# WeChatCV/WeDetect

Hardware: AMD Instinct MI355X
Metric: images/s at 640x640 (WeDetect-Base image tower + 80-class similarity + top-k/NMS) (higher is better)
Workload: dtype f32-equivalent: fp32 operands carried as fp16 hi+lo pairs, 3 fp16-MFMA passes per product, fp32 accumulate (fp16x3); similarity GEMM, dwconv, LN, post-process native f32

## Files before the change

__graft_entry__.py:

```python
import os
import sys

ROOT = os.path.dirname(os.path.abspath(__file__))
if ROOT not in sys.path:
    sys.path.insert(0, ROOT)


def build() -> None:
    from wedetect_amd import build as wb
    wb.build()
    import wedetect_amd.lib as lib
    import wedetect_amd.feed
    import wedetect_amd.tile
    import wedetect_amd.views
    import wedetect_amd.fold
    import wedetect_amd.best
    import wedetect_amd.sparse
    import wedetect_amd.topn
    import wedetect_amd.groups
    import wedetect_amd.exemplar
    import wedetect_amd.tune
    import wedetect_amd.track
    import wedetect_amd.detector
    import oracle.postprocess
    import oracle.ref_cpu
    print("built and loaded", lib.LIB_PATH)


def smoke() -> None:
    import numpy as np
    import torch
    from oracle import postprocess as opp
    from oracle import ref_cpu as orc
    from wedetect_amd import weights as W
    from wedetect_amd.arch import get_arch
    from wedetect_amd.engine import ImageTower
    from wedetect_amd.pack import pack

    assert torch.cuda.is_available(), "smoke() needs a HIP device"
    torch.cuda.set_device(0)
    arch, b, hw, npr = "tiny", 2, 128, 64
    sd_np = W.make_state_dict(arch, num_prompts=npr)
    tower = ImageTower(arch, pack(sd_np, arch), b, hw, hw)
    imgs = W.make_images(b, hw, hw)
    embed, boxes = tower.features(torch.from_numpy(imgs).cuda())
# ... 27 lines not shown
```

wedetect_amd/build.py:

```python
from __future__ import annotations

import os
import subprocess
import sys

HERE = os.path.dirname(os.path.abspath(__file__))
ROOT = os.path.dirname(HERE)
CSRC = os.path.join(HERE, "csrc")
LIB = os.path.join(HERE, "libwedetect_hip.so")
SOURCES = ["abi.hip", "conv_gemm.hip", "similarity_grouped.hip", "split_gemm.hip", "split_gemm_pre.hip", "split_gemm_p8.hip", "split_gemm_p4.hip", "split_gemm_conv.hip", "split_gemm_conv3.hip", "split_gemm_mlp.hip", "split_gemm_mlpw.hip", "probe.hip", "stem.hip", "elementwise.hip", "preprocess.hip", "text.hip", "bricks.hip", "evaluate.hip", "det_eval.hip", "postprocess.hip", "feed.hip", "tile.hip", "views.hip", "fold.hip", "best.hip", "sparse.hip", "topn.hip", "groups.hip", "exemplar.hip", "tune.hip", "track.hip"]
PUBLIC_HEADERS = ["wedetect_hip.h", "wedetect_hip_feed.h", "wedetect_hip_tile.h", "wedetect_hip_views.h", "wedetect_hip_fold.h", "wedetect_hip_best.h", "wedetect_hip_sparse.h", "wedetect_hip_topn.h", "wedetect_hip_groups.h", "wedetect_hip_exemplar.h", "wedetect_hip_tune.h", "wedetect_hip_track.h"]
HIPCC = os.environ.get("HIPCC", "/opt/rocm/bin/hipcc")
FLAGS = ["--offload-arch=gfx950", "-O3", "-std=c++17", "-fPIC", "-Wall", "-Wno-unused-function", "-Wno-inline-asm",
         "-I", os.path.join(ROOT, "include"), "-I", CSRC]
for _d in os.environ.get("WD_EXTRA_DEFINES", "").split():
    FLAGS.append("-D" + _d)
if os.environ.get("WD_DEBUG_ABLATIONS") == "1":
    FLAGS.append("-DWD_DEBUG_ABLATIONS")


def _headers():
    return [os.path.join(CSRC, f) for f in os.listdir(CSRC) if f.endswith(".h")] + [os.path.join(ROOT, "include", h) for h in PUBLIC_HEADERS]


def source_hash() -> str:
    import hashlib
    h = hashlib.sha256()
    files = sorted(os.path.join(CSRC, f) for f in os.listdir(CSRC) if f.endswith((".hip", ".h")))
    for f in files + [os.path.join(ROOT, "include", h) for h in PUBLIC_HEADERS]:
        h.update(os.path.basename(f).encode())
        h.update(open(f, "rb").read())
    return h.hexdigest()


# ... 112 lines not shown
```

wedetect_amd/csrc/split_gemm_mlpw.hip:

```cpp
#include <stdlib.h>
#include "split_epi_oct.h"
#include "split_mlp_epi.h"

namespace {

template <int C>
struct MW {
  static constexpr int H = 4 * C, BM = 128, HC = 128, NCH = H / HC;
  static constexpr int KT = 64, NKT = C / KT;
  static constexpr int XSLOT = BM * 256, NSLOT = 3;
  static constexpr int HOFF = NSLOT * XSLOT;
  static constexpr int LDS = HOFF + BM * 512;
  static constexpr int TN2 = C / 128;
  static constexpr int S1 = C / 16, S2 = H / 16;
  static_assert(C % 128 == 0 && NKT >= 2 && LDS <= 160 * 1024, "shape");
  static_assert(4 * 32 * EPI_LDT * 4 <= HOFF, "the epilogue patches reuse the ring");
};

struct MwArgs {
  const unsigned char* a;
  const unsigned char* w1;
  const unsigned char* w2;
  const float* b1;
  const float* b2;
// ... 40 lines not shown
    asm volatile("global_load_dwordx4 %0, %2, %3\n\tglobal_load_dwordx4 %1, %2, %3 offset:1024"
                 : "=&v"(hi), "=&v"(lo) : "v"(lane16), "s"(base) : "memory");
}
template <bool SAFE>
__device__ __forceinline__ void mw_bload(f32x4& d, unsigned voff, const float* base) {
  if constexpr (SAFE)
    asm volatile("s_nop 4\n\tglobal_load_dwordx4 %0, %1, %2" : "=&v"(d) : "v"(voff), "s"(base) : "memory");
  else
    asm volatile("global_load_dwordx4 %0, %1, %2" : "=&v"(d) : "v"(voff), "s"(base) : "memory");
}
#define MW_WAIT8_(N, A0, A1, A2, A3, A4, A5, A6, A7) \
  asm volatile("s_waitcnt vmcnt(" #N ")" : "+v"(A0), "+v"(A1), "+v"(A2), "+v"(A3), "+v"(A4), "+v"(A5), "+v"(A6), "+v"(A7) :: "memory")
#ifdef MW_EXPERIMENT_ALL0
#define MW_WAIT8(N, ...) MW_WAIT8_(0, __VA_ARGS__)
#else
#define MW_WAIT8(N, ...) MW_WAIT8_(N, __VA_ARGS__)
#endif

template <int C, int ABL = 0, bool PERSIST = false, bool FOLD = false>
__global__ void __launch_bounds__(256) fused_mlp_wide_kernel(const MwArgs q) {
  using P = MW<C>;
  constexpr int TN2 = P::TN2, NKT = P::NKT;
  static_assert(NKT % 2 == 0 && NKT >= 4, "K tiles alternate between two W1 fragment buffers");
  extern __shared__ __attribute__((aligned(16))) unsigned char smem_raw[];
  const int t = threadIdx.x, lane = t & 63;
  const int wave = __builtin_amdgcn_readfirstlane(t >> 6);
  int first_blk, seg_o, last_blk, seg_e;
  if (PERSIST) {
    const int b = blockIdx.x, xcd = b & 7, slot = b >> 3, per = gridDim.x >> 3;
    const long long t0 = (long long)q.nblk * xcd / 8, t1 = (long long)q.nblk * (xcd + 1) / 8;
    const long long units = (t1 - t0) * P::NCH;
    const long long u0 = t0 * P::NCH + units * slot / per, u1 = t0 * P::NCH + units * (slot + 1) / per;
    first_blk = (int)(u0 / P::NCH); seg_o = (int)(u0 - (long long)first_blk * P::NCH);
    last_blk = (int)(u1 / P::NCH); seg_e = (int)(u1 - (long long)last_blk * P::NCH);
  } else {
    int tile = blockIdx.x;
    const int nwg = gridDim.x, xcd = tile & 7, idx = tile >> 3;
    const int qq = nwg >> 3, r = nwg & 7;
    tile = (xcd < r ? xcd * (qq + 1) : r * (qq + 1) + (xcd - r) * qq) + idx;
    first_blk = tile; seg_o = 0; last_blk = tile + 1; seg_e = 0;
  }
  const int has_head = seg_e > 0, has_tail = seg_o > 0;
  const int full0 = first_blk + has_tail, nfull = last_blk - full0;
  const int nseg = has_head + nfull + has_tail;
  unsigned lds0 = (unsigned)(size_t)(__attribute__((address_space(3))) unsigned char*)smem_raw;

// ... 13 lines not shown
  const int r = lane & 31, hsel = lane >> 5, f = r & 15;
  const int xb = r * 256 + (((2 * hsel) ^ f) << 4);
  const int hb = r * 512 + (((2 * hsel) ^ f) << 4);
  const unsigned char* hbuf = smem_raw + P::HOFF;

  const unsigned lane16 = (unsigned)lane * 16u;
  const unsigned char* w1w_ = q.w1 + (size_t)wave * (P::S1 * 2048);
  const unsigned char* w2w_ = q.w2 + (size_t)(TN2 * wave) * (P::S2 * 2048);
  const unsigned char *w1w = w1w_, *w2w = w2w_;
  const unsigned bvoff = (unsigned)hsel * 16u;
  const float* b1p = q.b1 + wave * 32;
  const float* u1p = FOLD ? q.ln_u + wave * 32 : nullptr;

  using I0 = std::integral_constant<int, 0>;
  using I1 = std::integral_constant<int, 1>;

  for (int sg = 0; sg < nseg; ++sg) {
  const bool is_head = has_head && sg == 0;
  const bool is_tail = has_tail && sg == nseg - 1;
  const int blk = is_head ? last_blk : (is_tail ? first_blk : full0 + sg - has_head);
  const int c0 = is_tail ? seg_o : 0, c1 = is_head ? seg_e : P::NCH;
  const int m0 = blk * P::BM;
  arow = q.a + (size_t)m0 * (C * 4);
  MW_BARRIER();

  f32x16 out[4][TN2];
  if (PERSIST && is_tail) {
    const int prev = blockIdx.x - 8;
    if (t == 0) {
      while (__hip_atomic_load(q.flag + prev, __ATOMIC_RELAXED, __HIP_MEMORY_SCOPE_AGENT) != 1u) __builtin_amdgcn_s_sleep(8);
      __builtin_amdgcn_fence(__ATOMIC_ACQUIRE, "agent");
    }
    __syncthreads();
    const unsigned char* sb = reinterpret_cast<const unsigned char*>(q.park) + (size_t)prev * (4 * TN2 * 4 * 4096);
    const unsigned toff = (unsigned)t * 16u;
#pragma unroll
    for (int i = 0; i < 4; ++i) {
      f32x4 v[TN2][4];
#pragma unroll
      for (int jn = 0; jn < TN2; ++jn)
#pragma unroll
        for (int g = 0; g < 4; ++g) {
          MW_OPAQUE(sb);
          v[jn][g] = *reinterpret_cast<const f32x4*>(sb + toff);
          sb += 4096;
        }
// ... 23 lines not shown
  h8 wh[2][4], wl[2][4];
  h8 vh[2][TN2], vl[2][TN2];
  f32x4 bq[4];
  f32x4 uq[4] = {};
  typedef float f32x2_ __attribute__((ext_vector_type(2)));
  f32x2_ st[4] = {};

  auto load_w1_tile = [&](int j, int kt, int buf) {
    if ((ABL & 8) && (j > c0 || kt > 1)) return;
    const unsigned char* b = w1w + (size_t)(4 * j) * (P::S1 * 2048) + kt * 8192;
#pragma unroll
    for (int s = 0; s < 4; ++s) mw_wload<PERSIST>(wh[buf][s], wl[buf][s], lane16, b + s * 2048);
  };
  auto load_w2_step = [&](int S, int buf) {
    if ((ABL & 8) && S > 1) return;
    const unsigned char* b = w2w + (size_t)S * 2048;
#pragma unroll
    for (int jn = 0; jn < TN2; ++jn) mw_wload<PERSIST>(vh[buf][jn], vl[buf][jn], lane16, b + (size_t)jn * (P::S2 * 2048));
  };
  auto load_bias = [&](int j) {
    const float* b = b1p + j * P::HC;
#pragma unroll
    for (int g = 0; g < 4; ++g) mw_bload<PERSIST>(bq[g], bvoff, b + 8 * g);
    if constexpr (FOLD) {
      const float* u = u1p + j * P::HC;
#pragma unroll
      for (int g = 0; g < 4; ++g) mw_bload<PERSIST>(uq[g], bvoff, u + 8 * g);
    }
  };

  MW_OPAQUE(arow); MW_OPAQUE(w1w); MW_OPAQUE(w2w); MW_OPAQUE(b1p); MW_OPAQUE(lds0);
  issue_x(0, 0);
  issue_x(1, 1);
  load_w1_tile(c0, 0, 0);
  load_w1_tile(c0, 1, 1);
  load_bias(c0);
  if constexpr (FOLD) {
    const float* sp = q.ln_stats + 2 * (size_t)m0;
    MW_OPAQUE(sp);
#pragma unroll
    for (int i = 0; i < 4; ++i) {
      const unsigned so = (unsigned)(32 * i + r) * 8u;
      if constexpr (PERSIST) asm volatile("s_nop 4\n\tglobal_load_dwordx2 %0, %1, %2" : "=&v"(st[i]) : "v"(so), "s"(sp) : "memory");
      else asm volatile("global_load_dwordx2 %0, %1, %2" : "=&v"(st[i]) : "v"(so), "s"(sp) : "memory");
    }
    asm volatile("s_waitcnt vmcnt(0)" : "+v"(st[0]), "+v"(st[1]), "+v"(st[2]), "+v"(st[3]) :: "memory");
  } else {
    asm volatile("s_waitcnt vmcnt(0)" ::: "memory");
  }

  for (int j = c0; j < c1; ++j) {
    const int jn1 = j + 1 < c1 ? j + 1 : j;
    MW_OPAQUE(arow); MW_OPAQUE(w1w); MW_OPAQUE(w2w); MW_OPAQUE(b1p); MW_OPAQUE(lds0);
    f32x16 g1[4];
#pragma unroll
    for (int i = 0; i < 4; ++i)
#pragma unroll
      for (int e = 0; e < 16; ++e) g1[i][e] = 0.0f;

    auto ktile = [&](auto kt_c, auto buf_c, int slot) {
      constexpr int KT_ = decltype(kt_c)::value, BUF = decltype(buf_c)::value;
      if (!(ABL & 2)) {
#ifdef MW_EXPERIMENT_TILE_WAIT
        MW_WAIT8(MW_EXPERIMENT_TILE_WAIT, wh[BUF][0], wl[BUF][0], wh[BUF][1], wl[BUF][1], wh[BUF][2], wl[BUF][2], wh[BUF][3], wl[BUF][3]);
#else
        if constexpr (KT_ == 0 && TN2 == 2 && FOLD) MW_WAIT8(20, wh[BUF][0], wl[BUF][0], wh[BUF][1], wl[BUF][1], wh[BUF][2], wl[BUF][2], wh[BUF][3], wl[BUF][3]);
        else if constexpr (KT_ == 0 && TN2 == 2) MW_WAIT8(16, wh[BUF][0], wl[BUF][0], wh[BUF][1], wl[BUF][1], wh[BUF][2], wl[BUF][2], wh[BUF][3], wl[BUF][3]);
        else if constexpr (KT_ <= 1 && FOLD) MW_WAIT8(24, wh[BUF][0], wl[BUF][0], wh[BUF][1], wl[BUF][1], wh[BUF][2], wl[BUF][2], wh[BUF][3], wl[BUF][3]);
        else if constexpr (KT_ <= 1) MW_WAIT8(20, wh[BUF][0], wl[BUF][0], wh[BUF][1], wl[BUF][1], wh[BUF][2], wl[BUF][2], wh[BUF][3], wl[BUF][3]);
        else if constexpr (KT_ == NKT - 1) MW_WAIT8(8, wh[BUF][0], wl[BUF][0], wh[BUF][1], wl[BUF][1], wh[BUF][2], wl[BUF][2], wh[BUF][3], wl[BUF][3]);
        else MW_WAIT8(16, wh[BUF][0], wl[BUF][0], wh[BUF][1], wl[BUF][1], wh[BUF][2], wl[BUF][2], wh[BUF][3], wl[BUF][3]);
#endif
      }
      if (!(ABL & 4)) MW_BARRIER();
      {
        int s2 = slot + 2;
        if (s2 >= P::NSLOT) s2 -= P::NSLOT;
        issue_x(KT_ + 2 < NKT ? KT_ + 2 : KT_ + 2 - NKT, s2);
      }
      const unsigned char* xs = smem_raw + slot * P::XSLOT;
      const unsigned char* wnext = w1w + (size_t)(4 * j) * (P::S1 * 2048) + (KT_ + 2) * 8192;
      h8 xh[2][4], xl[2][4];
      auto read_x = [&](int ks, h8 (&fh)[4], h8 (&fl)[4]) {
#pragma unroll
        for (int i = 0; i < 4; ++i) {
          fh[i] = *reinterpret_cast<const h8*>(xs + i * 8192 + (xb ^ (ks * 64)));
          fl[i] = *reinterpret_cast<const h8*>(xs + i * 8192 + (xb ^ (ks * 64 + 16)));
        }
      };
      read_x(0, xh[0], xl[0]);
      __builtin_amdgcn_sched_barrier(0);
#pragma unroll
      for (int ks = 0; ks < 4; ++ks) {
        const int cb = ks & 1;
        if (ks < 3) read_x(ks + 1, xh[cb ^ 1], xl[cb ^ 1]);
#pragma unroll
        for (int i = 0; i < 4; ++i) g1[i] = __builtin_amdgcn_mfma_f32_32x32x16_f16(wl[BUF][ks], xh[cb][i], g1[i], 0, 0, 0);
#pragma unroll
        for (int i = 0; i < 4; ++i) g1[i] = __builtin_amdgcn_mfma_f32_32x32x16_f16(wh[BUF][ks], xl[cb][i], g1[i], 0, 0, 0);
#pragma unroll
        for (int i = 0; i < 4; ++i) g1[i] = __builtin_amdgcn_mfma_f32_32x32x16_f16(wh[BUF][ks], xh[cb][i], g1[i], 0, 0, 0);
        if (ks < 3) {
// ... 7 lines not shown
        __builtin_amdgcn_sched_barrier(0);
        if constexpr (KT_ + 2 < NKT) {
          if (!(ABL & 8)) mw_wload<PERSIST>(wh[BUF][ks], wl[BUF][ks], lane16, wnext + ks * 2048);
        }
      }
    };
    {
      int slot = 0;
      slot = ((j - c0) * (NKT % P::NSLOT)) % P::NSLOT;
      auto adv = [&]() { slot = slot + 1 == P::NSLOT ? 0 : slot + 1; };
      ktile(std::integral_constant<int, 0>{}, I0{}, slot); adv();
      ktile(std::integral_constant<int, 1>{}, I1{}, slot); adv();
      ktile(std::integral_constant<int, 2>{}, I0{}, slot); adv();
      ktile(std::integral_constant<int, 3>{}, I1{}, slot); adv();
      if constexpr (NKT == 8) {
        ktile(std::integral_constant<int, 4>{}, I0{}, slot); adv();
        ktile(std::integral_constant<int, 5>{}, I1{}, slot); adv();
        ktile(std::integral_constant<int, 6>{}, I0{}, slot); adv();
        ktile(std::integral_constant<int, 7>{}, I1{}, slot); adv();
      }
    }

    load_w2_step(8 * j, 0);
    load_w2_step(8 * j + 1, 1);
#ifdef MW_EXPERIMENT_ALL0
    asm volatile("s_waitcnt vmcnt(0)" : "+v"(bq[0]), "+v"(bq[1]), "+v"(bq[2]), "+v"(bq[3]) :: "memory");
#else
    asm volatile("s_waitcnt vmcnt(48)" : "+v"(bq[0]), "+v"(bq[1]), "+v"(bq[2]), "+v"(bq[3]) :: "memory");
#endif
    if constexpr (FOLD) asm volatile("" : "+v"(uq[0]), "+v"(uq[1]), "+v"(uq[2]), "+v"(uq[3]));

#pragma unroll
    for (int i = 0; i < 4; ++i) {
      u32x2 hi[4], lo[4];
#pragma unroll
      for (int g = 0; g < 4; ++g) {
        if (ABL & 1) {
          hi[g] = u32x2{__builtin_bit_cast(unsigned, g1[i][4 * g]), __builtin_bit_cast(unsigned, g1[i][4 * g + 1])};
          lo[g] = u32x2{__builtin_bit_cast(unsigned, g1[i][4 * g + 2]), __builtin_bit_cast(unsigned, g1[i][4 * g + 3])};
        } else {
          const f32x4 v = {g1[i][4 * g], g1[i][4 * g + 1], g1[i][4 * g + 2], g1[i][4 * g + 3]};
          f32x4 o;
#pragma unroll
          for (int e = 0; e < 4; ++e) {
            if constexpr (FOLD) o[e] = wd_gelu(fmaf(st[i][1], fmaf(-st[i][0], uq[g][e], v[e] * q.unscale1), bq[g][e]));
            else o[e] = wd_gelu(fmaf(v[e], q.unscale1, bq[g][e]));
          }
          if (q.hid_scale != 1.0f) o = o * q.hid_scale;
          split4(o, hi[g], lo[g]);
        }
      }
#pragma unroll
      for (int s = 0; s < 2; ++s) {
        h8 fh8, fl8;
        mc_epi_swap(hi, lo, s, fh8, fl8);
        const int grp = 4 * wave + 2 * s + hsel;
        unsigned char* hp = smem_raw + P::HOFF + (32 * i + r) * 512;
        *reinterpret_cast<h8*>(hp + (((2 * grp) ^ f) << 4)) = fh8;
        *reinterpret_cast<h8*>(hp + (((2 * grp + 1) ^ f) << 4)) = fl8;
      }
    }
    asm volatile("s_waitcnt lgkmcnt(0)" ::: "memory");
    MW_BARRIER();

    h8 hh[2][4], hl[2][4];
    auto read_h = [&](int ks, h8 (&fh)[4], h8 (&fl)[4]) {
#pragma unroll
      for (int i = 0; i < 4; ++i) {
        fh[i] = *reinterpret_cast<const h8*>(hbuf + i * 16384 + (hb ^ (ks * 64)));
        fl[i] = *reinterpret_cast<const h8*>(hbuf + i * 16384 + (hb ^ (ks * 64 + 16)));
      }
    };
    auto g2step = [&](auto ks_c, auto buf_c) {
      constexpr int KS = decltype(ks_c)::value, BUF = decltype(buf_c)::value;
      static_assert(TN2 == 4 || TN2 == 2, "wait operand lists");
      if constexpr (TN2 == 4) {
#define MW_W2WAIT(N) MW_WAIT8(N, vh[BUF][0], vl[BUF][0], vh[BUF][1], vl[BUF][1], vh[BUF][2], vl[BUF][2], vh[BUF][3], vl[BUF][3])
        if constexpr (KS <= 4) MW_W2WAIT(8); else if constexpr (KS == 5) MW_W2WAIT(16); else if constexpr (KS == 6) MW_W2WAIT(24); else if constexpr (FOLD) MW_W2WAIT(16); else MW_W2WAIT(12);
#undef MW_W2WAIT
      } else {
#ifdef MW_EXPERIMENT_ALL0
#define MW_W2WAIT(N) asm volatile("s_waitcnt vmcnt(0)" : "+v"(vh[BUF][0]), "+v"(vl[BUF][0]), "+v"(vh[BUF][1]), "+v"(vl[BUF][1]) :: "memory")
#else
#define MW_W2WAIT(N) asm volatile("s_waitcnt vmcnt(" #N ")" : "+v"(vh[BUF][0]), "+v"(vl[BUF][0]), "+v"(vh[BUF][1]), "+v"(vl[BUF][1]) :: "memory")
#endif
        if constexpr (KS <= 4) MW_W2WAIT(4); else if constexpr (KS == 5) MW_W2WAIT(12); else if constexpr (KS == 6) MW_W2WAIT(20); else if constexpr (FOLD) MW_W2WAIT(16); else MW_W2WAIT(12);
#undef MW_W2WAIT
      }
      if constexpr (KS == 0) {
        read_h(0, hh[0], hl[0]);
        __builtin_amdgcn_sched_barrier(0);
      }
      if constexpr (KS < 7) read_h(KS + 1, hh[BUF ^ 1], hl[BUF ^ 1]);
#pragma unroll
      for (int i = 0; i < 4; ++i)
#pragma unroll
        for (int jn = 0; jn < TN2; ++jn) out[i][jn] = __builtin_amdgcn_mfma_f32_32x32x16_f16(vl[BUF][jn], hh[BUF][i], out[i][jn], 0, 0, 0);
#pragma unroll
      for (int i = 0; i < 4; ++i)
#pragma unroll
        for (int jn = 0; jn < TN2; ++jn) out[i][jn] = __builtin_amdgcn_mfma_f32_32x32x16_f16(vh[BUF][jn], hl[BUF][i], out[i][jn], 0, 0, 0);
#pragma unroll
      for (int i = 0; i < 4; ++i)
#pragma unroll
        for (int jn = 0; jn < TN2; ++jn) out[i][jn] = __builtin_amdgcn_mfma_f32_32x32x16_f16(vh[BUF][jn], hh[BUF][i], out[i][jn], 0, 0, 0);
      if constexpr (KS < 7) {
#pragma unroll
        for (int u = 0; u < 8; ++u) {
          __builtin_amdgcn_sched_group_barrier(0x008, 1, 0);
          __builtin_amdgcn_sched_group_barrier(0x100, 1, 0);
        }
        __builtin_amdgcn_sched_group_barrier(0x008, 12 * TN2 - 8, 0);
      }
      __builtin_amdgcn_sched_barrier(0);
      if constexpr (KS < 6) load_w2_step(8 * j + KS + 2, BUF);
      if constexpr (KS == 4) load_w1_tile(jn1, 0, 0);
      if constexpr (KS == 5) load_w1_tile(jn1, 1, 1);
      if constexpr (KS == 6) load_bias(jn1);
    };
    g2step(std::integral_constant<int, 0>{}, I0{});
    g2step(std::integral_constant<int, 1>{}, I1{});
    g2step(std::integral_constant<int, 2>{}, I0{});
    g2step(std::integral_constant<int, 3>{}, I1{});
    g2step(std::integral_constant<int, 4>{}, I0{});
    g2step(std::integral_constant<int, 5>{}, I1{});
    g2step(std::integral_constant<int, 6>{}, I0{});
    g2step(std::integral_constant<int, 7>{}, I1{});
  }
  MW_WAIT8(0, wh[0][0], wl[0][0], wh[0][1], wl[0][1], wh[0][2], wl[0][2], wh[0][3], wl[0][3]);
  asm volatile("" : "+v"(wh[1][0]), "+v"(wl[1][0]), "+v"(wh[1][1]), "+v"(wl[1][1]), "+v"(wh[1][2]), "+v"(wl[1][2]), "+v"(wh[1][3]), "+v"(wl[1][3]));
  asm volatile("" : "+v"(bq[0]), "+v"(bq[1]), "+v"(bq[2]), "+v"(bq[3]));
  if constexpr (FOLD) asm volatile("" : "+v"(uq[0]), "+v"(uq[1]), "+v"(uq[2]), "+v"(uq[3]));
#pragma unroll
  for (int jn = 0; jn < TN2; ++jn) asm volatile("" : "+v"(vh[0][jn]), "+v"(vl[0][jn]), "+v"(vh[1][jn]), "+v"(vl[1][jn]));
  MW_BARRIER();

  if (PERSIST && is_head) {
    unsigned char* sb = reinterpret_cast<unsigned char*>(q.park) + (size_t)blockIdx.x * (4 * TN2 * 4 * 4096);
    const unsigned toff = (unsigned)t * 16u;
#pragma unroll
    for (int i = 0; i < 4; ++i)
#pragma unroll
      for (int jn = 0; jn < TN2; ++jn)
#pragma unroll
        for (int g = 0; g < 4; ++g) {
          MW_OPAQUE(sb);
          *reinterpret_cast<f32x4*>(sb + toff) = f32x4{out[i][jn][4 * g], out[i][jn][4 * g + 1], out[i][jn][4 * g + 2], out[i][jn][4 * g + 3]};
          sb += 4096;
        }
    asm volatile("s_waitcnt vmcnt(0)" ::: "memory");
    __syncthreads();
    if (t == 0) {
      __builtin_amdgcn_fence(__ATOMIC_RELEASE, "agent");
      asm volatile("s_waitcnt vmcnt(0)" ::: "memory");
      __hip_atomic_store(q.flag + blockIdx.x, 1u, __ATOMIC_RELAXED, __HIP_MEMORY_SCOPE_AGENT);
// ... 72 lines not shown
           nullptr, nullptr, 0, nullptr, nullptr};
  float* ws = static_cast<float*>(workspace);
  const long long wsf = workspace ? workspace_bytes / 4 : 0;
  hipStream_t st = static_cast<hipStream_t>(stream);
#ifdef WD_DEBUG_ABLATIONS
  if (const char* e = getenv("WD_MLPW_ABL")) {
    if (c != 512) return WD_ERR_UNSUPPORTED;
    switch (atoi(e)) {
      case 1: return launch_mlp_wide<512, 1>(q, st, ws, wsf);
      case 2: return launch_mlp_wide<512, 2>(q, st, ws, wsf);
      case 4: return launch_mlp_wide<512, 4>(q, st, ws, wsf);
      case 6: return launch_mlp_wide<512, 6>(q, st, ws, wsf);
      case 7: return launch_mlp_wide<512, 7>(q, st, ws, wsf);
      case 8: return launch_mlp_wide<512, 8>(q, st, ws, wsf);
      case 14: return launch_mlp_wide<512, 14>(q, st, ws, wsf);
      case 15: return launch_mlp_wide<512, 15>(q, st, ws, wsf);
      default: break;
    }
  }
#endif
  return c == 512 ? launch_mlp_wide<512>(q, st, ws, wsf) : launch_mlp_wide<256>(q, st, ws, wsf);
}

extern "C" int wd_mlp_fused_wide_ln(const void* d_split, int64_t rows, int32_t c, int32_t hidden, const void* w1g_frag,
                                    float w1_unscale, const float* v, const float* u, const float* ln_stats, const void* w2_frag,
                                    float w2_unscale, const float* b2, float* x, float hid_scale, uint32_t* range_flag,
                                    void* workspace, int64_t workspace_bytes, void* stream) {
  if (workspace && (!wd_aligned16(workspace) || workspace_bytes < 0)) return WD_ERR_BAD_ARG;
  if (!d_split || !w1g_frag || !w2_frag || !v || !u || !ln_stats || !b2 || !x) return WD_ERR_BAD_ARG;
  if (c != 256 || hidden != 4 * c) return WD_ERR_UNSUPPORTED;
  if (rows <= 0 || rows % 128 || rows / 128 > 0x7fffffffLL) return WD_ERR_UNSUPPORTED;
  if (!wd_aligned16(d_split) || !wd_aligned16(w1g_frag) || !wd_aligned16(w2_frag) || !wd_aligned16(v) || !wd_aligned16(u) ||
      !wd_aligned16(b2) || !wd_aligned16(x) || (reinterpret_cast<uintptr_t>(ln_stats) & 7u))
    return WD_ERR_BAD_ARG;
  if (!(w1_unscale > 0.f) || !(w2_unscale > 0.f) || !(hid_scale > 0.f)) return WD_ERR_BAD_ARG;
  MwArgs q{static_cast<const unsigned char*>(d_split), static_cast<const unsigned char*>(w1g_frag),
           static_cast<const unsigned char*>(w2_frag), v, b2, x, range_flag, (int)rows, w1_unscale, w2_unscale, hid_scale,
           nullptr, nullptr, 0, ln_stats, u};
  return launch_mlp_wide<256, 0, true>(q, static_cast<hipStream_t>(stream), static_cast<float*>(workspace), workspace ? workspace_bytes / 4 : 0);
}
```

wedetect_amd/engine.py:

```python
from __future__ import annotations

import contextlib
import copy
import math
import os
import warnings
import weakref
from typing import Dict, List, Optional, Sequence, Tuple

import numpy as np
import torch

from . import fold as FD
from . import lib as L
from .arch import ArchSpec, CLS_MID, EMBED_DIM, REG_MID, STRIDES, get_arch, level_sizes
from .pack import Packed


DEFAULT_PRECISION = "fp16x3"


def fold_layernorm_into_linear(w1: torch.Tensor, b1: torch.Tensor, gamma: torch.Tensor, beta: torch.Tensor):
    w64, g64 = w1.double(), gamma.double()
    w1g = (w64 * g64[None, :]).float().contiguous()
    u = w1g.double().sum(dim=1).float().contiguous()
    v = (w64 @ beta.double() + b1.double()).float().contiguous()
    return w1g, u, v


_DEVICE_STREAMS: Dict[str, Dict[str, list]] = {}


def device_streams(dev: torch.device, role: str, n: int = 1) -> List[torch.cuda.Stream]:
    pool = _DEVICE_STREAMS.setdefault(str(dev), {})
    if not pool:
        for r in ("post", "nh", "bb2"):
            pool[r] = [torch.cuda.Stream(device=dev)]
# ... 330 lines not shown
        return not (self._pipe_issue or self.force_tile_forms) or self.pipe_persist in ("1", family)

    def _fold_weights(self, q: str) -> None:
        if q + "w1g" in self.P.t:
            return
        self.P.t[q + "w1g"], self.P.t[q + "u"], self.P.t[q + "v"] = fold_layernorm_into_linear(
            self.P[q + "w1"], self.P[q + "b1"], self.P[q + "ln_w"], self.P[q + "ln_b"])

    def _prepare_fold(self) -> None:
        a = self.a
        stages = [i for i in range(4)
                  if self._fold_ok(i, self.precision == "fp16x3" and a.dims[i] % 8 == 0 and (i == 0 or a.dims[i - 1] % 8 == 0))]
        if not stages:
            return
        if self.ln_stats is None:
            rows = max(self.M[k] for k in range(4))
            blk = max(self.M[k] * (a.dims[k] // 32) for k in range(4) if a.dims[k] % 32 == 0)
            self.ln_part = torch.empty(2 * blk, dtype=torch.float32, device=self.dev)
            self.ln_stats = torch.empty(2 * rows, dtype=torch.float32, device=self.dev)
        if not torch.cuda.is_current_stream_capturing():
            for i in stages:
                for j in range(a.depths[i]):
                    self._fold_weights(f"s{i}.{j}.")

    def _fold_ok(self, i: int, pre: bool) -> bool:
        c = self.a.dims[i]
        if not (self.ln_fold and pre and self.precision == "fp16x3" and c % 32 == 0):
            return False
        if self.fuse_dwln == "1" or (self.fuse_dwln == "auto" and (c <= 128 or c in self.fuse_dwln_wide)):
            return False
        if self.fuse_mlp and L.mlp_fused_supported(self.M[i], c, 4 * c):
            return False
        if c in self.fuse_mlp_wide and L.mlp_wide_supported(self.M[i], c, 4 * c):
            return self.ln_fold_fused and c in L.MLP_WIDE_FOLD_WIDTHS
        return True

    def _mlp_fused_fold(self, q: str, i: int) -> None:
        c = self.a.dims[i]
        self._fold_weights(q)
        ws = []
        for name, (n_, k_) in ((q + "w1g", (4 * c, c)), (q + "w2", (c, 4 * c))):
            f_ = self.Wf.get(name)
            if f_ is None:
                s_ = self.Ws.get(name)
                if s_ is None:
                    wt = self.P[name]
                    s_ = self.Ws[name] = L.split_weights(wt.view(wt.shape[0], -1))
                f_ = self.Wf[name] = (L.mlp_wide_pack(s_[0], n_, k_), s_[1])
            ws.append(f_)
        sa, sh = self.sscale.get(q + "dw", 1.0), self.sscale.get(q + "hid", 1.0)
        if self._park_mlp is None:
            self._park_mlp = self.park if self.park is not None else torch.zeros(
                max(1, L.p8_workspace_bytes() // 4), dtype=torch.float32, device=self.dev)
        L.mlp_fused_wide_ln(self.tmp, self.M[i], c, 4 * c, (ws[0][0], ws[0][1] / sa), self.P[q + "v"], self.P[q + "u"], self.ln_stats,
                            (ws[1][0], ws[1][1] / sh), self.P[q + "b2"], self.x[i], hid_scale=sh, range_flag=self.range_flag,
                            workspace=self._park_mlp if self._persist_ok("mlp") else None)

    def _mlp_fused(self, q: str, i: int, wide: bool = False) -> None:
        c = self.a.dims[i]
        ws = []
        for name in (q + "w1", q + "w2"):
            s_ = self.Ws.get(name)
            if s_ is None:
                wt = self.P[name]
                s_ = self.Ws[name] = L.split_weights(wt.view(wt.shape[0], -1))
            if wide:
                f_ = self.Wf.get(name)
                if f_ is None:
                    n_, k_ = (4 * c, c) if name.endswith("w1") else (c, 4 * c)
                    f_ = self.Wf[name] = (L.mlp_wide_pack(s_[0], n_, k_), s_[1])
                s_ = f_
            ws.append(s_)
        sa, sh = self.sscale.get(q + "ln", 1.0), self.sscale.get(q + "hid", 1.0)
        kw = {}
        if wide:
            if self._park_mlp is None:
                self._park_mlp = self.park if self.park is not None else torch.zeros(
                    max(1, L.p8_workspace_bytes() // 4), dtype=torch.float32, device=self.dev)
            kw["workspace"] = self._park_mlp if self._persist_ok("mlp") else None
# ... 225 lines not shown
            cp = a.dims[i - 1]
            hp, wp = self.hw[i - 1]
            if pre and hp % 2 == 0 and wp % 2 == 0 and self.s2d_down:
                g_, b_ = self._ln_params(f"down{i}.ln_w", f"down{i}.ln_b", f"down{i}.ln")
                L.layernorm_rows_split_s2d(self.x[i - 1], self.tmp, g_, b_, B, hp, wp, cp)
                self._gemm(self.tmp, f"down{i}.w", f"down{i}.b", self.x[i], hin=h, win=w, cin=4 * cp, lda=4 * cp, n=c,
                           ldc=c, split_flags=fa, a_key=f"down{i}.ln")
            else:
                g_, b_ = self._ln_params(f"down{i}.ln_w", f"down{i}.ln_b", f"down{i}.ln" if pre else None)
                L.layernorm_rows(self.x[i - 1], self.tmp, g_, b_, self.M[i - 1], cp, split=pre)
                self._record(f"down{i}.ln", self.tmp[: self.M[i - 1] * cp])
                self._gemm(self.tmp, f"down{i}.w", f"down{i}.b", self.x[i], hin=hp, win=wp, cin=cp, lda=cp, kh=2, kw=2,
                           stride=2, pad=0, n=c, ldc=c, split_flags=fa, a_key=f"down{i}.ln" if pre else None)
        for j in range(a.depths[i]):
            q = f"s{i}.{j}."
            yield "dw"
            if self._fold_ok(i, pre) and not self.sscale.get(q + "fold_off"):
                self._prepare_fold()
                self._fold_weights(q)
                L.dwconv7_stats(self.x[i], self.P[q + "dw_w"], self.P[q + "dw_b"], self.tmp, self.ln_part, B, h, w, c,
                                scale=self.sscale.get(q + "dw", 1.0))
                L.ln_stats_finalize(self.ln_part, self.ln_stats, self.M[i], c)
                yield "mlp"
                if c in self.fuse_mlp_wide and L.mlp_wide_supported(self.M[i], c, 4 * c):
                    self._mlp_fused_fold(q, i)
                    continue
                self._conv(self.tmp, q + "w1g", q + "v", self.hid, hin=h, win=w, cin=c, lda=c, n=4 * c, ldc=4 * c,
                           act=L.ACT_GELU, split_flags=L.SPLIT_A | L.SPLIT_C, a_key=q + "dw", c_key=q + "hid",
                           ln_stats=self.ln_stats, ln_u=self.P[q + "u"])
                self._conv(self.hid, q + "w2", q + "b2", self.x[i], hin=h, win=w, cin=4 * c, lda=4 * c, n=c, ldc=c,
                           res=self.x[i], ldres=c, split_flags=fa, a_key=q + "hid")
                continue
            g_, b_ = self._ln_params(q + "ln_w", q + "ln_b", q + "ln" if pre else None)
            if c % 32 == 0 and (self.fuse_dwln == "1" or (self.fuse_dwln == "auto" and (c <= 128 or c in self.fuse_dwln_wide))):
                L.dwconv7_ln(self.x[i], self.P[q + "dw_w"], self.P[q + "dw_b"], self.tmp, g_, b_, B, h, w, c, split=pre)
            else:
                L.dwconv7(self.x[i], self.P[q + "dw_w"], self.P[q + "dw_b"], self.tmp, B, h, w, c)
                if self._calib is not None and self.ln_fold:
                    self._record(q + "dw", self.tmp[: self.M[i] * c])
                    d = self.tmp[: self.M[i] * c].view(self.M[i], c)
                    self._calib[q + "dw.mr"] = (d.mean(dim=1).abs() / d.std(dim=1, unbiased=False).clamp_min(1e-30)).max()
                L.layernorm_rows(self.tmp, self.tmp, g_, b_, self.M[i], c, split=pre)
            self._record(q + "ln", self.tmp[: self.M[i] * c])
            yield "mlp"
            if pre and self.fuse_mlp and L.mlp_fused_supported(self.M[i], c, 4 * c):
                self._mlp_fused(q, i)
                continue
            if pre and c in self.fuse_mlp_wide and L.mlp_wide_supported(self.M[i], c, 4 * c):
                self._mlp_fused(q, i, wide=True)
                continue
            self._conv(self.tmp, q + "w1", q + "b1", self.hid, hin=h, win=w, cin=c, lda=c, n=4 * c, ldc=4 * c,
                       act=L.ACT_GELU, split_flags=(L.SPLIT_A | L.SPLIT_C) if pre else 0,
                       a_key=q + "ln" if pre else None, c_key=q + "hid")
            self._conv(self.hid, q + "w2", q + "b2", self.x[i], hin=h, win=w, cin=4 * c, lda=4 * c, n=c, ldc=c,
                       res=self.x[i], ldres=c, split_flags=fa, a_key=q + "hid" if pre else None)

    def _bepc3(self, name: str, x, ldx: int, cin: int, hw: Tuple[int, int], out, cout: int, xkey: str, okey: str):
        bf = self._bep[name]
        c_ = bf["c_"]
        h, w = hw
        nb = self.a.neck_repeats // 2
        cat = bf["cat"]
        S = self._neck_split()
        fl = (L.SPLIT_A | L.SPLIT_C) if S else 0
        sfx = "s" if S else ""
        D = self._dag_on()

        def cv2():
            self._conv(x, f"{name}.cv2.w", f"{name}.cv2.b", cat[:, c_:], hin=h, win=w, cin=cin, lda=ldx, n=c_,
                       ldc=2 * c_, act=L.ACT_SILU, split_flags=fl, a_key=xkey, c_key=name + ".cat")
        ev_cv2 = None
# ... 1070 lines not shown
```

wedetect_amd/lib.py:

```python
from __future__ import annotations

import ctypes as C
import math
import os

import torch

_HERE = os.path.dirname(os.path.abspath(__file__))
LIB_PATH = os.environ.get("WEDETECT_LIB") or os.path.join(_HERE, "libwedetect_hip.so")

ACT_NONE, ACT_RELU, ACT_SILU, ACT_GELU = 0, 1, 2, 3
OUT_ROWS, OUT_DECONV2X2 = 0, 1
SPLIT_A, SPLIT_C = 1, 2
ABI_VERSION = 15
NMS_VANILLA, NMS_TORCHVISION, NMS_MMCV = 0, 1, 2
TV_TRICK_MAX_NUMEL = {"cpu": 4000, "cuda": 20000}
MMCV_SPLIT_THR = 10000

EXPORTS = (
    "wd_abi_version", "wd_strerror", "wd_sizeof_conv_gemm", "wd_conv_gemm", "wd_conv_gemm_tuned", "wd_conv_gemm_config", "wd_stem_patchify", "wd_dwconv7", "wd_dwconv7_variant",
    "wd_layernorm_rows", "wd_l2norm_rows", "wd_dfl_decode", "wd_topk_workspace_bytes", "wd_topk_capacity",
    "wd_topk_candidates", "wd_nms_workspace_bytes", "wd_nms_gather", "wd_retrieval_max",
    "wd_split_weights_bytes", "wd_split_weights", "wd_split_weights_padded", "wd_dwconv7_stats", "wd_ln_stats_finalize", "wd_conv_gemm_split", "wd_conv_gemm_split_ws", "wd_conv_gemm_split_config", "wd_layernorm_rows_split", "wd_layernorm_rows_split_s2d", "wd_letterbox_u8", "wd_retrieval_max_split", "wd_similarity_split", "wd_similarity_grouped", "wd_mlp_fused_wide_ln", "wd_text_embed", "wd_attention_small", "wd_recall_scratch_floats", "wd_recall_match",
    "wd_det_match_workspace_bytes", "wd_det_match_lds_bytes", "wd_det_match", "wd_det_sort", "wd_det_accumulate",
# ... 153 lines not shown
        p.seg_scale = (C.c_float * 3)(*[float(v) for v in seg[3]])
        p.seg_bias = (C.c_float * 3)(*[float(v) for v in seg[4]])
    if w_split is not None:
        if workspace is not None:
            check(LIB.wd_conv_gemm_split_ws(C.byref(p), _p(w_split[0]), float(w_split[1]), int(split_flags), int(split_cfg),
                                            _p(workspace), workspace.numel() * workspace.element_size(), int(k_splits),
                                            stream_ptr()), f"wd_conv_gemm_split_ws[{split_cfg}]")
            return
        check(LIB.wd_conv_gemm_split(C.byref(p), _p(w_split[0]), float(w_split[1]), int(split_flags), int(split_cfg),
                                     stream_ptr()),
              f"wd_conv_gemm_split[{split_cfg}]")
        return
    if tuned_cfg is not None:
        check(LIB.wd_conv_gemm_tuned(C.byref(p), int(tuned_cfg), stream_ptr()), f"wd_conv_gemm_tuned[{tuned_cfg}]")
        return
    check(LIB.wd_conv_gemm(C.byref(p), stream_ptr()), "wd_conv_gemm")


def mlp_fused_supported(rows: int, c: int, hidden: int) -> bool:
    return c == 128 and hidden == 512 and rows > 0 and rows % 128 == 0


MLP_WIDE_WIDTHS = (256, 512)
MLP_WIDE_FOLD_WIDTHS = (256,)


def mlp_wide_supported(rows: int, c: int, hidden: int) -> bool:
    return c in MLP_WIDE_WIDTHS and hidden == 4 * c and rows > 0 and rows % 128 == 0


def mlp_wide_pack(w_split: torch.Tensor, n: int, k: int) -> torch.Tensor:
    if n % 32 or k % 16 or w_split.numel() != n * k * 4:
        raise WedetectHipError(f"mlp_wide_pack: [{n}][{k}] is not a whole number of 32 x 16 fragments")
    v = w_split.view(n // 32, 32, k // 16, 2, 2, 16)
    return v.permute(0, 2, 4, 3, 1, 5).contiguous().view(-1)


def mlp_fused_wide(a_split, rows, c, hidden, w1_frag, b1, w2_frag, b2, x, hid_scale=1.0, range_flag=None, workspace=None) -> None:
    ws_bytes = 0 if workspace is None else workspace.numel() * workspace.element_size()
    check(LIB.wd_mlp_fused_wide(_p(a_split), rows, c, hidden, _p(w1_frag[0]), float(w1_frag[1]), _p(b1), _p(w2_frag[0]),
                                float(w2_frag[1]), _p(b2), _p(x), float(hid_scale), _p(range_flag), _p(workspace), ws_bytes,
                                stream_ptr()),
          "wd_mlp_fused_wide")


def mlp_fused_wide_ln(d_split, rows, c, hidden, w1g_frag, v, u, ln_stats, w2_frag, b2, x, hid_scale=1.0, range_flag=None, workspace=None) -> None:
    ws_bytes = 0 if workspace is None else workspace.numel() * workspace.element_size()
# ... 232 lines not shown
```

Before: 980.1.

## Extend LayerNorm-folded fused wide MLP kernel to 512-channel stages

Enables the LN-folded fused wide MLP path for C=512 blocks, which previously fell back to the non-folded path. This folds the LayerNorm into the first GEMM of those blocks and removes the separate normalized-activation pass. For C=512 the kernel loads the per-column u vector and per-row LN stats just in time, during the last K tile of each chunk, instead of keeping them resident. It also delays the second W2 prefetch so these loads fit, which is meant to limit register pressure. The 512 path is exposed through a new entry point and Python binding, and the fragment packing is hoisted to setup; the changed wait counts add some risk of memory-latency stalls.

```diff
diff --git a/__graft_entry__.py b/__graft_entry__.py
--- a/__graft_entry__.py
+++ b/__graft_entry__.py
@@ -21,6 +21,7 @@
     import wedetect_amd.exemplar
     import wedetect_amd.tune
     import wedetect_amd.track
+    import wedetect_amd.mlpw
     import wedetect_amd.detector
     import oracle.postprocess
     import oracle.ref_cpu
diff --git a/include/wedetect_hip_mlpw.h b/include/wedetect_hip_mlpw.h
--- /dev/null
+++ b/include/wedetect_hip_mlpw.h
@@ -0,0 +1,25 @@
+#ifndef WEDETECT_HIP_MLPW_H
+#define WEDETECT_HIP_MLPW_H
+
+#include <stdint.h>
+
+#include "wedetect_hip.h"
+
+#ifdef __cplusplus
+extern "C" {
+#endif
+
+#define WD_MLPW_ABI_VERSION 1
+
+int wd_mlpw_abi_version(void);
+
+int wd_mlp_wide_fold(const void* d_split, int64_t rows, int32_t c, int32_t hidden, const void* w1g_frag, float w1_unscale,
+                     const float* v, const float* u, const float* ln_stats, const void* w2_frag, float w2_unscale,
+                     const float* b2, float* x, float hid_scale, uint32_t* range_flag, void* workspace, int64_t workspace_bytes,
+                     void* stream);
+
+#ifdef __cplusplus
+}
+#endif
+
+#endif
diff --git a/wedetect_amd/build.py b/wedetect_amd/build.py
--- a/wedetect_amd/build.py
+++ b/wedetect_amd/build.py
@@ -9,7 +9,7 @@
 CSRC = os.path.join(HERE, "csrc")
 LIB = os.path.join(HERE, "libwedetect_hip.so")
 SOURCES = ["abi.hip", "conv_gemm.hip", "similarity_grouped.hip", "split_gemm.hip", "split_gemm_pre.hip", "split_gemm_p8.hip", "split_gemm_p4.hip", "split_gemm_conv.hip", "split_gemm_conv3.hip", "split_gemm_mlp.hip", "split_gemm_mlpw.hip", "probe.hip", "stem.hip", "elementwise.hip", "preprocess.hip", "text.hip", "bricks.hip", "evaluate.hip", "det_eval.hip", "postprocess.hip", "feed.hip", "tile.hip", "views.hip", "fold.hip", "best.hip", "sparse.hip", "topn.hip", "groups.hip", "exemplar.hip", "tune.hip", "track.hip"]
-PUBLIC_HEADERS = ["wedetect_hip.h", "wedetect_hip_feed.h", "wedetect_hip_tile.h", "wedetect_hip_views.h", "wedetect_hip_fold.h", "wedetect_hip_best.h", "wedetect_hip_sparse.h", "wedetect_hip_topn.h", "wedetect_hip_groups.h", "wedetect_hip_exemplar.h", "wedetect_hip_tune.h", "wedetect_hip_track.h"]
+PUBLIC_HEADERS = ["wedetect_hip.h", "wedetect_hip_feed.h", "wedetect_hip_tile.h", "wedetect_hip_views.h", "wedetect_hip_fold.h", "wedetect_hip_best.h", "wedetect_hip_sparse.h", "wedetect_hip_topn.h", "wedetect_hip_groups.h", "wedetect_hip_exemplar.h", "wedetect_hip_tune.h", "wedetect_hip_track.h", "wedetect_hip_mlpw.h"]
 HIPCC = os.environ.get("HIPCC", "/opt/rocm/bin/hipcc")
 FLAGS = ["--offload-arch=gfx950", "-O3", "-std=c++17", "-fPIC", "-Wall", "-Wno-unused-function", "-Wno-inline-asm",
          "-I", os.path.join(ROOT, "include"), "-I", CSRC]
diff --git a/wedetect_amd/csrc/split_gemm_mlpw.hip b/wedetect_amd/csrc/split_gemm_mlpw.hip
--- a/wedetect_amd/csrc/split_gemm_mlpw.hip
+++ b/wedetect_amd/csrc/split_gemm_mlpw.hip
@@ -86,6 +86,8 @@
   using P = MW<C>;
   constexpr int TN2 = P::TN2, NKT = P::NKT;
   static_assert(NKT % 2 == 0 && NKT >= 4, "K tiles alternate between two W1 fragment buffers");
+  constexpr bool JIT = FOLD && C == 512;
+  constexpr bool UBIAS = FOLD && !JIT;
   extern __shared__ __attribute__((aligned(16))) unsigned char smem_raw[];
   const int t = threadIdx.x, lane = t & 63;
   const int wave = __builtin_amdgcn_readfirstlane(t >> 6);
@@ -145,6 +147,7 @@
   const int c0 = is_tail ? seg_o : 0, c1 = is_head ? seg_e : P::NCH;
   const int m0 = blk * P::BM;
   arow = q.a + (size_t)m0 * (C * 4);
+  const float* stp = JIT ? q.ln_stats + 2 * (size_t)m0 : nullptr;
   MW_BARRIER();
 
   f32x16 out[4][TN2];
@@ -214,10 +217,17 @@
     const float* b = b1p + j * P::HC;
 #pragma unroll
     for (int g = 0; g < 4; ++g) mw_bload<PERSIST>(bq[g], bvoff, b + 8 * g);
-    if constexpr (FOLD) {
+    if constexpr (UBIAS) {
       const float* u = u1p + j * P::HC;
 #pragma unroll
       for (int g = 0; g < 4; ++g) mw_bload<PERSIST>(uq[g], bvoff, u + 8 * g);
+    }
+  };
+  auto load_fold_jit = [&](int j) {
+#pragma unroll
+    for (int g = 0; g < 4; ++g) {
+      mw_bload<PERSIST>(uq[g], bvoff, u1p + j * P::HC + 8 * g);
+      asm volatile("global_load_dwordx2 %0, %1, %2" : "=&v"(st[g]) : "v"((unsigned)(32 * g + r) * 8u), "s"(stp) : "memory");
     }
   };
 
@@ -227,7 +237,7 @@
   load_w1_tile(c0, 0, 0);
   load_w1_tile(c0, 1, 1);
   load_bias(c0);
-  if constexpr (FOLD) {
+  if constexpr (UBIAS) {
     const float* sp = q.ln_stats + 2 * (size_t)m0;
     MW_OPAQUE(sp);
 #pragma unroll
@@ -243,7 +253,7 @@
 
   for (int j = c0; j < c1; ++j) {
     const int jn1 = j + 1 < c1 ? j + 1 : j;
-    MW_OPAQUE(arow); MW_OPAQUE(w1w); MW_OPAQUE(w2w); MW_OPAQUE(b1p); MW_OPAQUE(lds0);
+    if constexpr (JIT) { MW_OPAQUE(u1p); MW_OPAQUE(stp); }  MW_OPAQUE(arow); MW_OPAQUE(w1w); MW_OPAQUE(w2w); MW_OPAQUE(b1p); MW_OPAQUE(lds0);
     f32x16 g1[4];
 #pragma unroll
     for (int i = 0; i < 4; ++i)
@@ -256,9 +266,9 @@
 #ifdef MW_EXPERIMENT_TILE_WAIT
         MW_WAIT8(MW_EXPERIMENT_TILE_WAIT, wh[BUF][0], wl[BUF][0], wh[BUF][1], wl[BUF][1], wh[BUF][2], wl[BUF][2], wh[BUF][3], wl[BUF][3]);
 #else
-        if constexpr (KT_ == 0 && TN2 == 2 && FOLD) MW_WAIT8(20, wh[BUF][0], wl[BUF][0], wh[BUF][1], wl[BUF][1], wh[BUF][2], wl[BUF][2], wh[BUF][3], wl[BUF][3]);
+        if constexpr (KT_ == 0 && TN2 == 2 && UBIAS) MW_WAIT8(20, wh[BUF][0], wl[BUF][0], wh[BUF][1], wl[BUF][1], wh[BUF][2], wl[BUF][2], wh[BUF][3], wl[BUF][3]);
         else if constexpr (KT_ == 0 && TN2 == 2) MW_WAIT8(16, wh[BUF][0], wl[BUF][0], wh[BUF][1], wl[BUF][1], wh[BUF][2], wl[BUF][2], wh[BUF][3], wl[BUF][3]);
-        else if constexpr (KT_ <= 1 && FOLD) MW_WAIT8(24, wh[BUF][0], wl[BUF][0], wh[BUF][1], wl[BUF][1], wh[BUF][2], wl[BUF][2], wh[BUF][3], wl[BUF][3]);
+        else if constexpr (KT_ <= 1 && UBIAS) MW_WAIT8(24, wh[BUF][0], wl[BUF][0], wh[BUF][1], wl[BUF][1], wh[BUF][2], wl[BUF][2], wh[BUF][3], wl[BUF][3]);
         else if constexpr (KT_ <= 1) MW_WAIT8(20, wh[BUF][0], wl[BUF][0], wh[BUF][1], wl[BUF][1], wh[BUF][2], wl[BUF][2], wh[BUF][3], wl[BUF][3]);
         else if constexpr (KT_ == NKT - 1) MW_WAIT8(8, wh[BUF][0], wl[BUF][0], wh[BUF][1], wl[BUF][1], wh[BUF][2], wl[BUF][2], wh[BUF][3], wl[BUF][3]);
         else MW_WAIT8(16, wh[BUF][0], wl[BUF][0], wh[BUF][1], wl[BUF][1], wh[BUF][2], wl[BUF][2], wh[BUF][3], wl[BUF][3]);
@@ -270,6 +280,7 @@
         if (s2 >= P::NSLOT) s2 -= P::NSLOT;
         issue_x(KT_ + 2 < NKT ? KT_ + 2 : KT_ + 2 - NKT, s2);
       }
+      if constexpr (JIT && KT_ == NKT - 1) load_fold_jit(j);
       const unsigned char* xs = smem_raw + slot * P::XSLOT;
       const unsigned char* wnext = w1w + (size_t)(4 * j) * (P::S1 * 2048) + (KT_ + 2) * 8192;
       h8 xh[2][4], xl[2][4];
@@ -323,16 +334,18 @@
     }
 
     load_w2_step(8 * j, 0);
-    load_w2_step(8 * j + 1, 1);
+    if constexpr (!JIT) load_w2_step(8 * j + 1, 1);
 #ifdef MW_EXPERIMENT_ALL0
     asm volatile("s_waitcnt vmcnt(0)" : "+v"(bq[0]), "+v"(bq[1]), "+v"(bq[2]), "+v"(bq[3]) :: "memory");
 #else
     asm volatile("s_waitcnt vmcnt(48)" : "+v"(bq[0]), "+v"(bq[1]), "+v"(bq[2]), "+v"(bq[3]) :: "memory");
 #endif
-    if constexpr (FOLD) asm volatile("" : "+v"(uq[0]), "+v"(uq[1]), "+v"(uq[2]), "+v"(uq[3]));
+    if constexpr (UBIAS) asm volatile("" : "+v"(uq[0]), "+v"(uq[1]), "+v"(uq[2]), "+v"(uq[3]));
+    if constexpr (JIT) MW_WAIT8(8, uq[0], uq[1], uq[2], uq[3], st[0], st[1], st[2], st[3]);
 
 #pragma unroll
     for (int i = 0; i < 4; ++i) {
+      if constexpr (JIT) if (i == 2) load_w2_step(8 * j + 1, 1);
       u32x2 hi[4], lo[4];
 #pragma unroll
       for (int g = 0; g < 4; ++g) {
@@ -377,7 +390,7 @@
       static_assert(TN2 == 4 || TN2 == 2, "wait operand lists");
       if constexpr (TN2 == 4) {
 #define MW_W2WAIT(N) MW_WAIT8(N, vh[BUF][0], vl[BUF][0], vh[BUF][1], vl[BUF][1], vh[BUF][2], vl[BUF][2], vh[BUF][3], vl[BUF][3])
-        if constexpr (KS <= 4) MW_W2WAIT(8); else if constexpr (KS == 5) MW_W2WAIT(16); else if constexpr (KS == 6) MW_W2WAIT(24); else if constexpr (FOLD) MW_W2WAIT(16); else MW_W2WAIT(12);
+        if constexpr (KS <= 4) MW_W2WAIT(8); else if constexpr (KS == 5) MW_W2WAIT(16); else if constexpr (KS == 6) MW_W2WAIT(24); else if constexpr (UBIAS) MW_W2WAIT(16); else MW_W2WAIT(12);
 #undef MW_W2WAIT
       } else {
 #ifdef MW_EXPERIMENT_ALL0
@@ -385,7 +398,7 @@
 #else
 #define MW_W2WAIT(N) asm volatile("s_waitcnt vmcnt(" #N ")" : "+v"(vh[BUF][0]), "+v"(vl[BUF][0]), "+v"(vh[BUF][1]), "+v"(vl[BUF][1]) :: "memory")
 #endif
-        if constexpr (KS <= 4) MW_W2WAIT(4); else if constexpr (KS == 5) MW_W2WAIT(12); else if constexpr (KS == 6) MW_W2WAIT(20); else if constexpr (FOLD) MW_W2WAIT(16); else MW_W2WAIT(12);
+        if constexpr (KS <= 4) MW_W2WAIT(4); else if constexpr (KS == 5) MW_W2WAIT(12); else if constexpr (KS == 6) MW_W2WAIT(20); else if constexpr (UBIAS) MW_W2WAIT(16); else MW_W2WAIT(12);
 #undef MW_W2WAIT
       }
       if constexpr (KS == 0) {
@@ -431,7 +444,7 @@
   MW_WAIT8(0, wh[0][0], wl[0][0], wh[0][1], wl[0][1], wh[0][2], wl[0][2], wh[0][3], wl[0][3]);
   asm volatile("" : "+v"(wh[1][0]), "+v"(wl[1][0]), "+v"(wh[1][1]), "+v"(wl[1][1]), "+v"(wh[1][2]), "+v"(wl[1][2]), "+v"(wh[1][3]), "+v"(wl[1][3]));
   asm volatile("" : "+v"(bq[0]), "+v"(bq[1]), "+v"(bq[2]), "+v"(bq[3]));
-  if constexpr (FOLD) asm volatile("" : "+v"(uq[0]), "+v"(uq[1]), "+v"(uq[2]), "+v"(uq[3]));
+  if constexpr (UBIAS) asm volatile("" : "+v"(uq[0]), "+v"(uq[1]), "+v"(uq[2]), "+v"(uq[3]));
 #pragma unroll
   for (int jn = 0; jn < TN2; ++jn) asm volatile("" : "+v"(vh[0][jn]), "+v"(vl[0][jn]), "+v"(vh[1][jn]), "+v"(vl[1][jn]));
   MW_BARRIER();
@@ -550,13 +563,13 @@
   return c == 512 ? launch_mlp_wide<512>(q, st, ws, wsf) : launch_mlp_wide<256>(q, st, ws, wsf);
 }
 
-extern "C" int wd_mlp_fused_wide_ln(const void* d_split, int64_t rows, int32_t c, int32_t hidden, const void* w1g_frag,
-                                    float w1_unscale, const float* v, const float* u, const float* ln_stats, const void* w2_frag,
-                                    float w2_unscale, const float* b2, float* x, float hid_scale, uint32_t* range_flag,
-                                    void* workspace, int64_t workspace_bytes, void* stream) {
+namespace {
+int mlp_wide_ln_entry(bool wide512, const void* d_split, int64_t rows, int32_t c, int32_t hidden, const void* w1g_frag, float w1_unscale,
+                      const float* v, const float* u, const float* ln_stats, const void* w2_frag, float w2_unscale, const float* b2,
+                      float* x, float hid_scale, uint32_t* range_flag, void* workspace, int64_t workspace_bytes, void* stream) {
   if (workspace && (!wd_aligned16(workspace) || workspace_bytes < 0)) return WD_ERR_BAD_ARG;
   if (!d_split || !w1g_frag || !w2_frag || !v || !u || !ln_stats || !b2 || !x) return WD_ERR_BAD_ARG;
-  if (c != 256 || hidden != 4 * c) return WD_ERR_UNSUPPORTED;
+  if ((c != 256 && !(wide512 && c == 512)) || hidden != 4 * c) return WD_ERR_UNSUPPORTED;
   if (rows <= 0 || rows % 128 || rows / 128 > 0x7fffffffLL) return WD_ERR_UNSUPPORTED;
   if (!wd_aligned16(d_split) || !wd_aligned16(w1g_frag) || !wd_aligned16(w2_frag) || !wd_aligned16(v) || !wd_aligned16(u) ||
       !wd_aligned16(b2) || !wd_aligned16(x) || (reinterpret_cast<uintptr_t>(ln_stats) & 7u))
@@ -565,5 +578,28 @@
   MwArgs q{static_cast<const unsigned char*>(d_split), static_cast<const unsigned char*>(w1g_frag),
            static_cast<const unsigned char*>(w2_frag), v, b2, x, range_flag, (int)rows, w1_unscale, w2_unscale, hid_scale,
            nullptr, nullptr, 0, ln_stats, u};
-  return launch_mlp_wide<256, 0, true>(q, static_cast<hipStream_t>(stream), static_cast<float*>(workspace), workspace ? workspace_bytes / 4 : 0);
-}
+  float* ws = static_cast<float*>(workspace);
+  const long long wsf = workspace ? workspace_bytes / 4 : 0;
+  hipStream_t st = static_cast<hipStream_t>(stream);
+  return c == 512 ? launch_mlp_wide<512, 0, true>(q, st, ws, wsf) : launch_mlp_wide<256, 0, true>(q, st, ws, wsf);
+}
+}
+
+extern "C" int wd_mlp_fused_wide_ln(const void* d_split, int64_t rows, int32_t c, int32_t hidden, const void* w1g_frag,
+                                    float w1_unscale, const float* v, const float* u, const float* ln_stats, const void* w2_frag,
+                                    float w2_unscale, const float* b2, float* x, float hid_scale, uint32_t* range_flag,
+                                    void* workspace, int64_t workspace_bytes, void* stream) {
+  return mlp_wide_ln_entry(false, d_split, rows, c, hidden, w1g_frag, w1_unscale, v, u, ln_stats, w2_frag, w2_unscale, b2, x, hid_scale,
+                           range_flag, workspace, workspace_bytes, stream);
+}
+
+#include "wedetect_hip_mlpw.h"
+extern "C" int wd_mlpw_abi_version(void) { return WD_MLPW_ABI_VERSION; }
+
+extern "C" int wd_mlp_wide_fold(const void* d_split, int64_t rows, int32_t c, int32_t hidden, const void* w1g_frag, float w1_unscale,
+                                const float* v, const float* u, const float* ln_stats, const void* w2_frag, float w2_unscale,
+                                const float* b2, float* x, float hid_scale, uint32_t* range_flag, void* workspace,
+                                int64_t workspace_bytes, void* stream) {
+  return mlp_wide_ln_entry(true, d_split, rows, c, hidden, w1g_frag, w1_unscale, v, u, ln_stats, w2_frag, w2_unscale, b2, x, hid_scale,
+                           range_flag, workspace, workspace_bytes, stream);
+}
diff --git a/wedetect_amd/engine.py b/wedetect_amd/engine.py
--- a/wedetect_amd/engine.py
+++ b/wedetect_amd/engine.py
@@ -13,6 +13,7 @@
 
 from . import fold as FD
 from . import lib as L
+from . import mlpw as MLPW
 from .arch import ArchSpec, CLS_MID, EMBED_DIM, REG_MID, STRIDES, get_arch, level_sizes
 from .pack import Packed
 
@@ -389,6 +390,8 @@
             for i in stages:
                 for j in range(a.depths[i]):
                     self._fold_weights(f"s{i}.{j}.")
+                    if self._mlp_wide_on(i):
+                        self._wide_fold_frags(f"s{i}.{j}.", a.dims[i])
 
     def _fold_ok(self, i: int, pre: bool) -> bool:
         c = self.a.dims[i]
@@ -398,12 +401,15 @@
             return False
         if self.fuse_mlp and L.mlp_fused_supported(self.M[i], c, 4 * c):
             return False
-        if c in self.fuse_mlp_wide and L.mlp_wide_supported(self.M[i], c, 4 * c):
+        if self._mlp_wide_on(i):
             return self.ln_fold_fused and c in L.MLP_WIDE_FOLD_WIDTHS
         return True
 
-    def _mlp_fused_fold(self, q: str, i: int) -> None:
+    def _mlp_wide_on(self, i: int) -> bool:
         c = self.a.dims[i]
+        return c in self.fuse_mlp_wide and L.mlp_wide_supported(self.M[i], c, 4 * c)
+
+    def _wide_fold_frags(self, q: str, c: int) -> list:
         self._fold_weights(q)
         ws = []
         for name, (n_, k_) in ((q + "w1g", (4 * c, c)), (q + "w2", (c, 4 * c))):
@@ -415,13 +421,19 @@
                     s_ = self.Ws[name] = L.split_weights(wt.view(wt.shape[0], -1))
                 f_ = self.Wf[name] = (L.mlp_wide_pack(s_[0], n_, k_), s_[1])
             ws.append(f_)
+        return ws
+
+    def _mlp_fused_fold(self, q: str, i: int) -> None:
+        c = self.a.dims[i]
+        ws = self._wide_fold_frags(q, c)
         sa, sh = self.sscale.get(q + "dw", 1.0), self.sscale.get(q + "hid", 1.0)
         if self._park_mlp is None:
             self._park_mlp = self.park if self.park is not None else torch.zeros(
                 max(1, L.p8_workspace_bytes() // 4), dtype=torch.float32, device=self.dev)
-        L.mlp_fused_wide_ln(self.tmp, self.M[i], c, 4 * c, (ws[0][0], ws[0][1] / sa), self.P[q + "v"], self.P[q + "u"], self.ln_stats,
-                            (ws[1][0], ws[1][1] / sh), self.P[q + "b2"], self.x[i], hid_scale=sh, range_flag=self.range_flag,
-                            workspace=self._park_mlp if self._persist_ok("mlp") else None)
+        fn = L.mlp_fused_wide_ln if c == 256 else MLPW.mlp_wide_fold
+        fn(self.tmp, self.M[i], c, 4 * c, (ws[0][0], ws[0][1] / sa), self.P[q + "v"], self.P[q + "u"], self.ln_stats,
+           (ws[1][0], ws[1][1] / sh), self.P[q + "b2"], self.x[i], hid_scale=sh, range_flag=self.range_flag,
+           workspace=self._park_mlp if self._persist_ok("mlp") else None)
 
     def _mlp_fused(self, q: str, i: int, wide: bool = False) -> None:
         c = self.a.dims[i]
@@ -693,7 +705,7 @@
                                 scale=self.sscale.get(q + "dw", 1.0))
                 L.ln_stats_finalize(self.ln_part, self.ln_stats, self.M[i], c)
                 yield "mlp"
-                if c in self.fuse_mlp_wide and L.mlp_wide_supported(self.M[i], c, 4 * c):
+                if self._mlp_wide_on(i):
                     self._mlp_fused_fold(q, i)
                     continue
                 self._conv(self.tmp, q + "w1g", q + "v", self.hid, hin=h, win=w, cin=c, lda=c, n=4 * c, ldc=4 * c,
@@ -717,7 +729,7 @@
             if pre and self.fuse_mlp and L.mlp_fused_supported(self.M[i], c, 4 * c):
                 self._mlp_fused(q, i)
                 continue
-            if pre and c in self.fuse_mlp_wide and L.mlp_wide_supported(self.M[i], c, 4 * c):
+            if pre and self._mlp_wide_on(i):
                 self._mlp_fused(q, i, wide=True)
                 continue
             self._conv(self.tmp, q + "w1", q + "b1", self.hid, hin=h, win=w, cin=c, lda=c, n=4 * c, ldc=4 * c,
diff --git a/wedetect_amd/lib.py b/wedetect_amd/lib.py
--- a/wedetect_amd/lib.py
+++ b/wedetect_amd/lib.py
@@ -199,7 +199,7 @@
 
 
 MLP_WIDE_WIDTHS = (256, 512)
-MLP_WIDE_FOLD_WIDTHS = (256,)
+MLP_WIDE_FOLD_WIDTHS = (256, 512)
 
 
 def mlp_wide_supported(rows: int, c: int, hidden: int) -> bool:
diff --git a/wedetect_amd/mlpw.py b/wedetect_amd/mlpw.py
--- /dev/null
+++ b/wedetect_amd/mlpw.py
@@ -0,0 +1,37 @@
+from __future__ import annotations
+
+import ctypes as C
+
+from . import lib as L
+
+MLPW_ABI_VERSION = 1
+WIDTHS = (256, 512)
+
+EXPORTS = ("wd_mlpw_abi_version", "wd_mlp_wide_fold")
+
+
+def _bind():
+    lib = L.LIB
+    for name in EXPORTS:
+        if not hasattr(lib, name):
+            raise L.WedetectHipMissing(f"{L.LIB_PATH} does not export {name}; rebuild (python -m wedetect_amd.build)")
+    vp, i32, i64, f32 = C.c_void_p, C.c_int32, C.c_int64, C.c_float
+    lib.wd_mlpw_abi_version.restype = C.c_int
+    lib.wd_mlp_wide_fold.argtypes = [vp, i64, i32, i32, vp, f32, vp, vp, vp, vp, f32, vp, vp, f32, vp, vp, i64, vp]
+    if lib.wd_mlpw_abi_version() != MLPW_ABI_VERSION:
+        raise L.WedetectHipMissing(f"mlpw ABI mismatch: library {lib.wd_mlpw_abi_version()} vs binding {MLPW_ABI_VERSION}; rebuild")
+    return lib
+
+
+LIB = _bind()
+
+
+def supported(rows: int, c: int, hidden: int) -> bool:
+    return c in WIDTHS and hidden == 4 * c and rows > 0 and rows % 128 == 0
+
+
+def mlp_wide_fold(d_split, rows, c, hidden, w1g_frag, v, u, ln_stats, w2_frag, b2, x, hid_scale=1.0, range_flag=None, workspace=None) -> None:
+    ws_bytes = 0 if workspace is None else workspace.numel() * workspace.element_size()
+    L.check(LIB.wd_mlp_wide_fold(L._p(d_split), rows, c, hidden, L._p(w1g_frag[0]), float(w1g_frag[1]), L._p(v), L._p(u), L._p(ln_stats),
+                                 L._p(w2_frag[0]), float(w2_frag[1]), L._p(b2), L._p(x), float(hid_scale), L._p(range_flag),
+                                 L._p(workspace), ws_bytes, L.stream_ptr()), "wd_mlp_wide_fold")
```

New measurement: 981.5 (median of 3 runs). Within noise of the previous version (+0.1%).
